# nelilepo/timetabling-ga-mpi-openmp

Hardware: AMD Instinct MI355X
Metric: fitness evals/sec (hcv+scv), pop 64K, 400-event instance; 1/2/4/8 GPUs (higher is better)
Workload: dtype i32; 1 GPU; med instance E=400 R=10 F=5 S=200 (seeded synthetic, medium01-size), population 65536 per GPU, one tt_eval (hcv+scv+feasible+penalty) per step; pop_per_gpu=65536, global_pop=65536, kernel=eval_tile5_w8, parallelism=dp1 (independent population shards)

## Files before the change

### timetabling-ga-mpi-openmp_amd/csrc/tt_eval.hip

```cpp
#include <algorithm>
#include <type_traits>
#include <utility>
#include <vector>

#include "tt_internal.h"

namespace ttga {

typedef __attribute__((address_space(4))) const uint32_t ConstU32;
typedef __attribute__((address_space(4))) const int32_t ConstI32;
typedef __attribute__((address_space(3))) unsigned long long LdsU64;


__device__ __forceinline__ int bcnt_acc(uint32_t x, int acc) {
    int r;
    asm("v_bcnt_u32_b32 %0, %1, %2" : "=v"(r) : "v"(x), "v"(acc));
    return r;
}
__device__ __forceinline__ int popc_acc(uint64_t x, int acc) {
    int r, t;
    asm("v_bcnt_u32_b32 %0, %1, %2" : "=v"(t) : "v"((uint32_t)x), "v"(acc));
    asm("v_bcnt_u32_b32 %0, %1, %2" : "=v"(r) : "v"((uint32_t)(x >> 32)), "v"(t));
    return r;
}
// ... 141 lines not shown
__device__ __forceinline__ int run_scv(const uint8_t* my, const uint32_t* p, int cnt) {
    constexpr int K = N <= 16 ? KMAX : 1;
    constexpr int ST = K * N / 2;
    const int steps = cnt / K;
    int sc = 0;
    if constexpr (KMAX == 1) {
        const ConstU32* q = (const ConstU32*)p;
        uint32_t cur[N / 2];
#pragma unroll
        for (int j = 0; j < N / 2; ++j) cur[j] = q[j];
        for (int i = 0; i < cnt; ++i) {
            const int in = i + 1 < cnt ? i + 1 : i;
            uint32_t nxt[N / 2];
#pragma unroll
            for (int j = 0; j < N / 2; ++j) nxt[j] = q[in * (N / 2) + j];
            uint32_t sl[N];
#pragma unroll
            for (int j = 0; j < N; ++j) sl[j] = my[(cur[j >> 1] >> (16 * (j & 1))) & 0xFFFFu];
            uint64_t m = 0;
#pragma unroll
            for (int j = 0; j < N; ++j) m |= 1ull << (sl[j] & 63);
            sc += mask_terms<GAP>(m);
#pragma unroll
            for (int j = 0; j < N / 2; ++j) cur[j] = nxt[j];
        }
        return sc;
    }
    const ConstU32* q = (const ConstU32*)p;
    if (steps > 0) {
        int i = 0;
        uint32_t ra[ST], rb[ST];
        sload_rec<ST>(q, ra);
        while (true) {
            sload_rec<ST>(q + (i + 1 < steps ? i + 1 : i) * ST, rb);
            sc += students_scv<N, K, GAP>(my, ra);
            keep_rec<ST>(rb);
            if (++i == steps) break;
            sload_rec<ST>(q + (i + 1 < steps ? i + 1 : i) * ST, ra);
            sc += students_scv<N, K, GAP>(my, rb);
            keep_rec<ST>(ra);
            if (++i == steps) break;
        }
    }
    if constexpr (K == 2) {
        if (cnt & 1) {
            uint32_t r[N / 2];
            sload_rec<N / 2>(q + steps * ST, r);
            sc += students_scv<N, 1, GAP>(my, r);
        }
    }
    return sc;
}
__device__ __noinline__ int run_scv_any(const uint8_t* my, const ConstU32* p, int cnt, int n, bool gap) {
    int sc = 0;
    for (int i = 0; i < cnt; ++i) {
        uint64_t m = 0;
        for (int j = 0; j < n / 2; ++j) {
            const uint32_t d = p[i * (n / 2) + j];
            m |= 1ull << (my[d & 0xFFFFu] & 63);
            m |= 1ull << (my[d >> 16] & 63);
        }
        sc += gap ? mask_scv_gap(m) : mask_scv(m);
    }
    return sc;
}
template <int KMAX, bool GAP = false>
__device__ __forceinline__ int lane_scv_runs(const uint8_t* my, const DevProblem& pb, int r0, int r1) {
    const ConstI32* runs = (const ConstI32*)pb.srun;
    int sc = 0;
    for (int k = r0; k < r1; ++k) {
        const int n = runs[4 * k], off = runs[4 * k + 1], cnt = runs[4 * k + 2];
        const uint32_t* p = pb.sid + off;
        switch (n) {
#define TT_RUN(N) case N: sc += run_scv<N, KMAX, GAP>(my, p, cnt); break;
            TT_RUN(2) TT_RUN(4) TT_RUN(6) TT_RUN(8) TT_RUN(10) TT_RUN(12) TT_RUN(14) TT_RUN(16)
            TT_RUN(18) TT_RUN(20) TT_RUN(22) TT_RUN(24) TT_RUN(26) TT_RUN(28) TT_RUN(30) TT_RUN(32)
#undef TT_RUN
            default: sc += run_scv_any(my, (const ConstU32*)p, cnt, n, GAP); break;
        }
    }
    return sc;
}

#ifndef TT_EVAL_ABLATE
#define TT_EVAL_ABLATE 0
#endif
__host__ __device__ inline int t5_cnt_bytes(int R) {
    return kSlots * ((R + 1) / 2) * 4;
}

struct Tile5Layout {
    int SP, WS;
    size_t tile_bytes, off_ws, off_part, bytes;
};

__host__ __device__ inline Tile5Layout tile5_layout(int E, int R, int NW, bool DB = false) {
    Tile5Layout L;
    int sp = (E + 1 + 3) & ~3;
    if (((sp >> 2) & 1) == 0) sp += 4;
    L.SP = sp;
    const int ew64 = (E + 63) / 64;
    const int cntb = t5_cnt_bytes(R);
    L.WS = (kSlots * ew64 * 8 + cntb + 15) & ~15;
    L.tile_bytes = ((size_t)64 * sp + 15) & ~(size_t)15;
    L.off_ws = (DB ? 2 : 1) * L.tile_bytes;
    L.off_part = L.off_ws + (size_t)NW * L.WS;
    L.bytes = L.off_part + 4 * (size_t)(NW * 64 + 64);
    return L;
}

template <int NW>
__device__ __forceinline__ void tile_dma(const uint8_t* src, uint8_t* dst, int np, int E, int SP, int wv, int lane) {
    const int qd = E >> 2;
    const __amdgpu_buffer_rsrc_t rs = __builtin_amdgcn_make_buffer_rsrc((void*)src, 0, np * E, 0x00020000);
    for (int r = wv; r < np; r += NW) {
        if (lane < qd)
            __builtin_amdgcn_raw_ptr_buffer_load_lds(rs, (__attribute__((address_space(3))) void*)(dst + r * SP), 4,
                                                     4 * lane, r * E, 0, 0);
        if (lane + 64 < qd)
            __builtin_amdgcn_raw_ptr_buffer_load_lds(rs, (__attribute__((address_space(3))) void*)(dst + r * SP + 256),
                                                     4, 4 * lane + 256, r * E, 0, 0);
    }
}

template <int NW>
__device__ __forceinline__ void image_dma(const uint8_t* img, int bytes, uint8_t* dst, int wv, int lane) {
    const __amdgpu_buffer_rsrc_t rs = __builtin_amdgcn_make_buffer_rsrc((void*)img, 0, bytes, 0x00020000);
    for (int k = wv; k < (bytes >> 8); k += NW)
        __builtin_amdgcn_raw_ptr_buffer_load_lds(rs, (__attribute__((address_space(3))) void*)(dst + 256 * k), 4,
                                                 4 * lane, 256 * k, 0, 0);
}

template <int EWC, int PK, int TP, typename PossT>
__device__ __forceinline__ void t5_load_inv(const uint8_t* img, int lane, uint64_t (*cup)[EWC], uint64_t* pcup,
                                            uint32_t* ps, PossT* poss, int* sn) {
    constexpr int F = TP == 1 ? EWC : EWC - 1;
    const uint64_t* c = (const uint64_t*)img + lane;
    const uint8_t* ev = img + 512 * t5_img_corr_rows(EWC, TP);
#pragma unroll
    for (int k = 0; k < t5_packed_rows(EWC, TP); ++k) pcup[k] = c[64 * (F * (F + 1) / 2 + k)];
#pragma unroll
    for (int r = 0; r < EWC; ++r) {
#pragma unroll
        for (int w = 0; w < EWC; ++w) cup[r][w] = (w >= r && w < F) ? c[64 * (r * F - r * (r - 1) / 2 + w - r)] : 0ull;
        if constexpr (PK == 1) {
            ps[r] = ((const uint32_t*)ev)[64 * r + lane];
        } else {
            poss[r] = ((const PossT*)ev)[64 * r + lane];
            sn[r] = ((const int*)(ev + EWC * 64 * sizeof(PossT)))[64 * r + lane];
        }
    }
}

#ifdef TT_T5_STAMP
constexpr int kT5Launches = 8, kT5MaxBlocks = 16384, kT5Words = 10;
__device__ unsigned long long g_t5_stamp[kT5Launches * kT5MaxBlocks * kT5Words];
#endif

__device__ __forceinline__ uint32_t mad_u16_hi(uint32_t a, uint32_t b, uint32_t c) {
    uint32_t d;
    asm("v_mad_u32_u16 %0, %1, %2, %3 op_sel:[0,1,0,0]" : "=v"(d) : "v"(a), "v"(b), "v"(c));
    return d;
}

constexpr uint32_t kT5ClrBias = 0x8000u;
constexpr size_t kT5ClrReach = 0x10000u + kT5ClrBias;
constexpr int t5_clear_max(int EWC, int PK) {
    return (kSlots * EWC * 8 + kSlots * (PK == 1 ? 8 : PK == 2 ? 16 : 32) * 4 + 15) / 256;
}
template <int MAXF>
__device__ __forceinline__ void t5_clear_pieces(uint32_t m0v, uint32_t skip) {
    uint32_t keep;
    asm volatile("s_mov_b32 %[keep], m0\n"
                 "s_mov_b32 m0, %[base]\n"
                 "s_getpc_b64 vcc\n"
                 "s_add_u32 vcc_lo, vcc_lo, %[skip]\n"
                 "s_addc_u32 vcc_hi, vcc_hi, 0\n"
                 "s_setpc_b64 vcc\n"
                 ".set tt_clr_k, %c[n]\n"
                 ".rept %c[n]\n"
                 ".set tt_clr_k, tt_clr_k-1\n"
                 "ds_write_addtid_b32 %[z] offset:tt_clr_k*256\n"
                 ".endr\n"
                 "s_branch .Ltt_clr_end%=\n"
                 ".set tt_clr_k, %c[n]\n"
                 ".rept %c[n]\n"
                 ".set tt_clr_k, tt_clr_k-1\n"
                 "ds_write_addtid_b32 %[z] offset:tt_clr_k*256+%c[bias]\n"
                 ".endr\n"
                 ".Ltt_clr_end%=:\n"
                 "s_mov_b32 m0, %[keep]\n"
                 "s_nop 0"
                 : [keep] "=&s"(keep)
                 : [base] "s"(m0v), [skip] "s"(skip), [z] "v"(0u), [n] "i"(MAXF), [bias] "i"(kT5ClrBias)
                 : "memory", "scc", "vcc");
}

constexpr int kT5PrioLane = 3;
constexpr uint32_t kT5PrioW = 0x00112233u;
template <int EWC, int NW, int PK, bool DB = false, int TP = 1>
__global__ __launch_bounds__(64 * NW, 4) void eval_tile5_kernel(DevProblem pb, const uint8_t* __restrict__ slot,
                                                              const uint8_t* __restrict__ room, int P,
                                                              int32_t* __restrict__ hcv_out,
                                                              int32_t* __restrict__ scv_out,
                                                              uint8_t* __restrict__ feas_out,
                                                              int32_t* __restrict__ pen_out, int ablate_arg) {
    extern __shared__ __attribute__((aligned(16))) uint8_t lds[];
    const int ablate = TT_EVAL_ABLATE ? ablate_arg : (ablate_arg & 3);
    constexpr int NT = 64 * NW;
#ifdef TT_T5_STAMP
    unsigned long long* st_rec =
        g_t5_stamp + ((size_t)((ablate_arg >> 8) & (kT5Launches - 1)) * kT5MaxBlocks + (blockIdx.x % kT5MaxBlocks)) * kT5Words;
    if (threadIdx.x == 0) {
        const unsigned long long t0 = __builtin_amdgcn_s_memrealtime();
        unsigned hw, xcc;
        asm volatile("s_getreg_b32 %0, hwreg(HW_REG_HW_ID)" : "=s"(hw));
        asm volatile("s_getreg_b32 %0, hwreg(HW_REG_XCC_ID)" : "=s"(xcc));
        st_rec[0] = t0;
        st_rec[1] = ((unsigned long long)xcc << 32) | hw;
    }
#endif
    const int E = pb.E, R = pb.R;
    const int lane = threadIdx.x & 63, wv = wave_id();
    const Tile5Layout L = tile5_layout(E, R, NW, DB);
    const int SP = L.SP;
    uint8_t* tile = lds;
    uint8_t* ws = lds + L.off_ws + (size_t)wv * L.WS;
    uint64_t* B = (uint64_t*)ws;
    uint32_t* cnt = (uint32_t*)(B + kSlots * EWC);
    int32_t* part = (int32_t*)(lds + L.off_part);
    int32_t* hq = part + NW * 64;
    const int tiles = (P + 63) / 64;
    const bool last_partial = E < 64 * EWC;
    const int RW = (R + 1) / 2;
    constexpr int CLRF = t5_clear_max(EWC, PK);
    const uint32_t ws_a = (uint32_t)__builtin_amdgcn_readfirstlane((int)lds_addr(ws));
    const bool ws_hi = ws_a >= 0x10000u;
    const uint32_t clr_m0 = ws_hi ? ws_a - kT5ClrBias : ws_a;
    const uint32_t clr_skip = 12u + 8u * (uint32_t)(CLRF - min(L.WS >> 8, CLRF)) + (ws_hi ? 8u * CLRF + 4u : 0u);

    using PossT = typename std::conditional<PK == 0, uint64_t, uint32_t>::type;
    uint64_t inv_cup[EWC][EWC];
    uint64_t inv_pcup[TP == 1 ? 1 : t5_packed_rows(EWC, TP)];
    PossT inv_poss[EWC];
    uint32_t inv_ps[EWC];
    int inv_sn[EWC];
    auto load_inv = [&](const uint8_t* img) { t5_load_inv<EWC, PK, TP, PossT>(img, lane, inv_cup, inv_pcup, inv_ps, inv_poss, inv_sn); };
    const bool img_lds = DB && (size_t)pb.t5_img_bytes <= L.tile_bytes;
    const ConstI32* ptab = (const ConstI32*)pb.srun_part;
    const int pbase = srun_part_base(NW);
    const int r0 = ptab[pbase + wv], r1 = ptab[pbase + wv + 1];
    const bool wide = (E & 15) == 0 && (((uintptr_t)slot) & 15) == 0;
    const int qpr = E >> 4;
    const uint32_t qinv = ((1u << 20) + (uint32_t)qpr - 1) / (uint32_t)max(qpr, 1);
    constexpr int TPL = 64 / TP;
    const uint32_t tcol = 64 * (EWC - 1) + ((lane & (TPL - 1)) + 64 * (EWC - 1) < E ? (lane & (TPL - 1)) : 0);
    const uint32_t pb0 = lds_addr(B) + 8 * (lane / TPL);

    if constexpr (DB) {
        if (threadIdx.x < 64) lds[threadIdx.x * SP + E] = 63;
        if (blockIdx.x < tiles)
            tile_dma<NW>(slot + (long)blockIdx.x * 64 * E, lds, (int)min(64L, (long)P - (long)blockIdx.x * 64), E, SP,
                         wv, lane);
        if (img_lds) {
            image_dma<NW>(pb.t5_img, pb.t5_img_bytes, lds + L.tile_bytes, wv, lane);
            asm volatile("s_waitcnt vmcnt(0)" ::: "memory");
            __syncthreads();
            load_inv(lds + L.tile_bytes);
            __syncthreads();
        } else {
            load_inv(pb.t5_img);
        }
        if (threadIdx.x < 64) lds[L.tile_bytes + threadIdx.x * SP + E] = 63;
    }
    auto stage = [&](const uint8_t* src, int np) {
        if (wide) {
            const uint4* s16 = (const uint4*)src;
#pragma unroll 2
            for (int w = threadIdx.x; w < np * qpr; w += NT) {
                const int r = (int)(((uint32_t)w * qinv) >> 20), c = w - r * qpr;
                const uint4 v = s16[w];
                uint32_t* d = (uint32_t*)(tile + r * SP + 16 * c);
                d[0] = v.x; d[1] = v.y; d[2] = v.z; d[3] = v.w;
            }
        } else {
#pragma unroll 1
            for (int r = wv; r < np; r += NW)
#pragma unroll 1
                for (int c = lane; c < E; c += 64) tile[r * SP + c] = src[(long)r * E + c];
        }
        if (threadIdx.x < 64) tile[threadIdx.x * SP + E] = 63;
    };
    if constexpr (!DB) {
        if (blockIdx.x < tiles)
            stage(slot + (long)blockIdx.x * 64 * E, (int)min(64L, (long)P - (long)blockIdx.x * 64));
        load_inv(pb.t5_img);
    }
    int it = 0;
    for (int tl = blockIdx.x; tl < tiles; tl += gridDim.x, ++it) {
        const long p0 = (long)tl * 64;
        const int np = (int)min((long)64, (long)P - p0);
        const uint8_t* src = slot + p0 * E;
        if constexpr (DB) {
            tile = lds + (it & 1) * L.tile_bytes;
            if (!(img_lds && it == 0)) {
                asm volatile("s_waitcnt vmcnt(0)" ::: "memory");
                __syncthreads();
            }
            const int tn = tl + gridDim.x;
            if (tn < tiles)
                tile_dma<NW>(slot + (long)tn * 64 * E, lds + ((it + 1) & 1) * L.tile_bytes,
                             (int)min(64L, (long)P - (long)tn * 64), E, SP, wv, lane);
        } else {
            if (it > 0) {
                __syncthreads();
                stage(src, np);
            }
            __syncthreads();
        }

        uint32_t lsp;
        asm volatile("v_mul_u32_u24 %0, %1, %2" : "=v"(lsp) : "v"(lane), "s"(SP));
        __builtin_amdgcn_s_setprio(kT5PrioLane);
        const int sc = (!(ablate & 1) && r0 < r1) ? lane_scv_runs<1>(tile + lsp, pb, r0, r1) : 0;
        part[wv * 64 + lane] = sc;

        const int nq = (ablate & 2) ? 0 : np;
        uint32_t pfn[EWC];
        const __amdgpu_buffer_rsrc_t rrs =
            __builtin_amdgcn_make_buffer_rsrc((void*)(room + p0 * E), 0, 64 * E, 0x00020000);
        auto load_row = [&](int q, uint32_t* dst) {
#pragma unroll
            for (int r = 0; r < EWC; ++r)
                dst[r] = (!last_partial || r < EWC - 1 || lane + 64 * r < E)
                             ? (uint32_t)__builtin_amdgcn_raw_buffer_load_b8(rrs, lane + 64 * r, q * E, 0)
                             : 0u;
        };
        if (wv < nq) load_row(wv, pfn);
        for (int q = wv; q < nq; q += NW) {
            const uint32_t pr = (kT5PrioW >> (4 * min((q - wv) / NW, 7))) & 3u;
            if (pr == 0) __builtin_amdgcn_s_setprio(0);
            else if (pr == 1) __builtin_amdgcn_s_setprio(1);
            else if (pr == 2) __builtin_amdgcn_s_setprio(2);
            else __builtin_amdgcn_s_setprio(3);
            uint32_t rv[EWC], sv[EWC];
#pragma unroll
            for (int r = 0; r < EWC; ++r) rv[r] = pfn[r];
            const uint8_t* rs = tile + q * SP;
#pragma unroll
            for (int r = 0; r < EWC; ++r)
                sv[r] = (!last_partial || r < EWC - 1 || lane + 64 * r < E) ? rs[lane + 64 * r] : 0u;
            uint32_t ts = 0;
            if constexpr (TP > 1) ts = rs[tcol];
            if (q + NW < nq) load_row(q + NW, pfn);
            uint32_t smax = 0, rmax = 0;
#pragma unroll
            for (int r = 0; r < EWC; ++r) { smax = max(smax, sv[r]); rmax = max(rmax, rv[r]); }
            const bool any_bad = wave_any(smax >= (uint32_t)kSlots || rmax >= (uint32_t)R);
            int h = 0, last = 0;
            if (!any_bad) {
                uint32_t row[EWC];
#pragma unroll
                for (int r = 0; r < EWC; ++r) row[r] = lds_addr(B) + __umul24(sv[r], (uint32_t)(EWC * 8));
                if (!(ablate & 32)) {
                    t5_clear_pieces<CLRF>(clr_m0, clr_skip);
                    *(uint32_t*)(ws + L.WS - 256 + 4 * lane) = 0u;
                }
                __builtin_amdgcn_fence(__ATOMIC_RELEASE, "wavefront");
                __builtin_amdgcn_wave_barrier();
                __builtin_amdgcn_fence(__ATOMIC_ACQUIRE, "wavefront");
#pragma unroll
                for (int r = 0; r < EWC; ++r) {
                    if (r < EWC - 1 || !last_partial || lane + 64 * r < E) {
                        const uint32_t s = sv[r], ro = rv[r];
                        if (!(ablate & 8))
                            __hip_atomic_fetch_or((LdsU64*)(uintptr_t)row[r] + r, 1ull << lane, __ATOMIC_RELAXED,
                                                  __HIP_MEMORY_SCOPE_AGENT);
                        if (!(ablate & 16)) {
                            uint32_t* c = (uint32_t*)((uint8_t*)cnt + ((__umul24(s, (uint32_t)(2 * RW)) + (ro & ~1u)) << 1));
                            const uint32_t sh = ro << 4;
                            h += (int)__builtin_amdgcn_ubfe(atomicAdd(c, 1u << (sh & 31u)), sh, 16);
                        }
                        const bool last_slot = (kLastSlotMask >> s) & 1ull;
                        if constexpr (PK == 1) {
                            h += (int)__builtin_amdgcn_ubfe(inv_ps[r], ro, 1);
                            last = (int)mad_u16_hi((uint32_t)(kLastSlotMask >> s) & 1u, inv_ps[r], (uint32_t)last);
                        } else {
                            h += (int)(((inv_poss[r] >> ro) & 1u) ^ 1u);
                            last += last_slot ? inv_sn[r] : 0;
                        }
                    }
                }
                __builtin_amdgcn_fence(__ATOMIC_RELEASE, "wavefront");
                __builtin_amdgcn_wave_barrier();
                __builtin_amdgcn_fence(__ATOMIC_ACQUIRE, "wavefront");
                if (!(ablate & 4)) {
                    if constexpr (TP == 1)
                        corr_words<0, EWC>(row, inv_cup, h);
                    else
                        corr_words_tp<0, EWC, TP>(row, pb0 + __umul24(ts, (uint32_t)(EWC * 8)), inv_cup, inv_pcup, h);
                }
                if (!wave_any(h >= 1024 || last >= 1024)) {
                    const uint32_t t = (uint32_t)wave_sum((h << 16) | last);
                    h = (int)(t >> 16);
                    last = (int)(t & 0xFFFFu);
                } else {
                    h = wave_sum(h);
                    last = wave_sum(last);
                }
                __builtin_amdgcn_fence(__ATOMIC_RELEASE, "wavefront");
                __builtin_amdgcn_wave_barrier();
                __builtin_amdgcn_fence(__ATOMIC_ACQUIRE, "wavefront");
            }
            if (lane == 0) {
                hq[q] = any_bad ? -1 : h;
                part[wv * 64 + q] += last;
            }
        }
        __syncthreads();
        if (wv == 0 && lane < np) {
            const long p = p0 + lane;
            const int h = hq[lane];
            if (h < 0) {
                hcv_out[p] = -1; scv_out[p] = -1; feas_out[p] = 0; pen_out[p] = -1;
            } else {
                int s2 = 0;
#pragma unroll
                for (int w = 0; w < NW; ++w) s2 += part[w * 64 + lane];
                hcv_out[p] = h;
                scv_out[p] = s2;
                feas_out[p] = h == 0 ? 1 : 0;
                pen_out[p] = h == 0 ? s2 : 1000000 + h;
            }
        }
    }
#ifdef TT_T5_STAMP
    if ((threadIdx.x & 63) == 0 && (threadIdx.x >> 6) < kT5Words - 2)
        st_rec[2 + (threadIdx.x >> 6)] = __builtin_amdgcn_s_memrealtime();
#endif
}

template <int NWL>
__global__ __launch_bounds__(64 * NWL) void eval_lanes_kernel(DevProblem pb, const uint8_t* __restrict__ slot, int P,
                                                              int32_t* __restrict__ scv_part) {
    extern __shared__ __attribute__((aligned(16))) uint8_t lds[];
    constexpr int NT = 64 * NWL;
    const int E = pb.E;
    const int lane = threadIdx.x & 63, wv = wave_id();
    int sp = (E + 1 + 3) & ~3;
    if (((sp >> 2) & 1) == 0) sp += 4;
    const int SP = sp;
    uint8_t* tile = lds;
    int32_t* part = (int32_t*)(lds + (((size_t)64 * SP + 15) & ~(size_t)15));
    const int tiles = (P + 63) / 64;
    const ConstI32* ptab = (const ConstI32*)pb.srun_part;
    const int pbase = srun_part_base(NWL);
    const int r0 = ptab[pbase + wv], r1 = ptab[pbase + wv + 1];
    const bool wide = (E & 15) == 0 && (((uintptr_t)slot) & 15) == 0;
    const int qpr = E >> 4;
    const uint64_t qinv = ((1ull << 32) + (uint64_t)qpr - 1) / (uint64_t)max(qpr, 1);

    for (int tl = blockIdx.x; tl < tiles; tl += gridDim.x) {
        const long p0 = (long)tl * 64;
        const int np = (int)min((long)64, (long)P - p0);
        __syncthreads();
        const uint8_t* src = slot + p0 * E;
        if (wide) {
            const uint4* s16 = (const uint4*)src;
#pragma unroll 2
            for (int w = threadIdx.x; w < np * qpr; w += NT) {
                const int r = (int)(((uint64_t)(uint32_t)w * qinv) >> 32), c = w - r * qpr;
                const uint4 v = s16[w];
                uint32_t* d = (uint32_t*)(tile + r * SP + 16 * c);
                d[0] = gap_slots4(v.x); d[1] = gap_slots4(v.y); d[2] = gap_slots4(v.z); d[3] = gap_slots4(v.w);
            }
        } else {
#pragma unroll 1
            for (int r = wv; r < np; r += NWL)
#pragma unroll 1
                for (int c = lane; c < E; c += 64) {
                    const uint8_t v = src[(long)r * E + c];
                    tile[r * SP + c] = gap_slot(v);
                }
        }
        if (threadIdx.x < 64) tile[threadIdx.x * SP + E] = 63;
        __syncthreads();
        const int sc = r0 < r1 ? lane_scv_runs<2, true>(tile + lane * SP, pb, r0, r1) : 0;
        part[wv * 64 + lane] = sc;
        __syncthreads();
        if (wv == 0 && lane < np) {
            int s2 = 0;
#pragma unroll
            for (int w = 0; w < NWL; ++w) s2 += part[w * 64 + lane];
            scv_part[p0 + lane] = s2;
        }
    }
}

struct CorrLayout {
    int NWV, BST, NB, EPL;
    size_t off_cnt, off_sl, WSI, off_acc, off_red, bytes;
};

__host__ __device__ inline CorrLayout corr_layout(int E, int R, int EW64, int NB) {
    CorrLayout L;
    const int pairs = (EW64 + 1) / 2;
    L.NWV = pairs < 16 ? pairs : 16;
    L.EPL = (E + 64 * L.NWV - 1) / (64 * L.NWV);
    L.BST = EW64 | 1;
    L.off_cnt = (size_t)kSlots * L.BST * 8;
    L.off_sl = L.off_cnt + (size_t)((kSlots * R + 1) / 2) * 4;
    L.WSI = (L.off_sl + (size_t)E + 15) & ~(size_t)15;
    L.NB = NB;
    L.off_acc = (size_t)NB * L.WSI;
    L.off_red = L.off_acc + (size_t)NB * 16;
    L.bytes = L.off_red + (size_t)NB * 2 * 64 * 4;
    return L;
}

constexpr int kCorrMaxEPL = 4;

template <int N, int OFF>
// ... 321 lines not shown
        std::vector<unsigned long long> z(sizeof(g_t5_stamp) / 8, 0ull);
        TT_HIP(hipMemcpyToSymbol(HIP_SYMBOL(g_t5_stamp), z.data(), sizeof(g_t5_stamp)));
    }
    return kT5Launches * kT5MaxBlocks;
}
#endif

extern "C" int tt_eval_variant(const tt_problem* p, const uint8_t* slot, const uint8_t* room, int P, int32_t* hcv,
                               int32_t* scv, uint8_t* feasible, int32_t* penalty, int variant, void* stream) {
    int rc = check_pop_args(p, P, slot, room);
    if (rc) return rc;
    if (P > 0 && (!hcv || !scv || !feasible || !penalty)) { set_error("null output buffer"); return TT_ERR_INVALID; }
    const int ablate = variant >> 4;
    variant &= 15;
    if (variant != 0 && variant != 2 && variant != 7 && variant != 8 && variant != 13) {
        set_error("unknown eval variant (0 auto, 2 block, 7/8 tile5, 13 wide)");
        return TT_ERR_INVALID;
    }
    if (P == 0) return TT_OK;
    rc = use_device(p);
    if (rc) return rc;
    hipStream_t st = (hipStream_t)stream;
    const int E = p->E, R = p->R;
    if (variant == 0) variant = auto_variant(p);
    if (variant == 13) {
        if (!wide_fits(p)) { set_error("instance outside the wide eval path"); return TT_ERR_LIMIT; }
        const int EW64 = p->dev.EW64;
        const int tiles = (P + 63) / 64;
        {
            const size_t lds_l = lanes_lds_bytes(E);
            auto launch_l = [&](auto kern) -> int {
                int per_cu = 0;
                TT_HIP(hipOccupancyMaxActiveBlocksPerMultiprocessor(&per_cu, kern, 1024, lds_l));
                per_cu = std::min(per_cu, lds_resident_limit(lds_l));
                const int grid = std::min(tiles, std::max(1, per_cu) * p->num_cus);
                hipLaunchKernelGGL(kern, dim3(grid), dim3(1024), lds_l, st, p->dev, slot, P, scv);
                return TT_OK;
            };
            rc = launch_l(eval_lanes_kernel<16>);
            if (rc) return rc;
        }
        if (ablate & 4) return check_hip(hipGetLastError(), "tt_eval launch");
        const int NB = corr_nb(E, R, EW64);
        const CorrLayout CL = corr_layout(E, R, EW64, NB);
        auto launch = [&](auto kern) -> int {
            int per_cu = 0;
            TT_HIP(hipOccupancyMaxActiveBlocksPerMultiprocessor(&per_cu, kern, 64 * CL.NWV, CL.bytes));
            per_cu = std::min(per_cu, lds_resident_limit(CL.bytes));
            const long batches = ((long)P + NB - 1) / NB;
            const int grid = (int)std::min<long>(batches, (long)std::max(1, per_cu) * p->num_cus);
            hipLaunchKernelGGL(kern, dim3(grid), dim3(64 * CL.NWV), CL.bytes, st, p->dev, slot, room, P, hcv, scv,
                               feasible, penalty, ablate);
            return TT_OK;
        };
        if (CL.EPL <= 2)
            rc = NB == 8 ? launch(eval_corr_kernel<8, 2>) : NB == 4 ? launch(eval_corr_kernel<4, 2>) : launch(eval_corr_kernel<2, 2>);
        else
            rc = NB == 8 ? launch(eval_corr_kernel<8, kCorrMaxEPL>)
                 : NB == 4 ? launch(eval_corr_kernel<4, kCorrMaxEPL>) : launch(eval_corr_kernel<2, kCorrMaxEPL>);
        if (rc) return rc;
    } else if (variant == 7 || variant == 8) {
        const int NW = variant == 7 ? 4 : 8;
        const Tile5Layout L0 = tile5_layout(E, R, NW, false), L1 = tile5_layout(E, R, NW, true);
        const bool db_ok = (E & 3) == 0 && (((uintptr_t)slot) & 3) == 0 && L1.bytes <= 160 * 1024 &&
                           L1.off_part <= kT5ClrReach;
        if (p->dev.EW64 > 7 || L0.bytes > 160 * 1024 || L0.off_part > kT5ClrReach || E > 32767) {
            set_error("instance too large for the tile5 kernel");
            return TT_ERR_LIMIT;
        }
        const int pk = t5_pk(R, p->max_sn), tp = t5_tp(E);
        const int tiles = (P + 63) / 64;
        auto occupancy = [&](auto kern, size_t bytes, bool two) -> int {
            std::atomic<int>& c = const_cast<tt_problem*>(p)->t5_occ[NW == 8][two];
            int per_cu = c.load(std::memory_order_relaxed);
            if (per_cu >= 0) return per_cu;
            if (hipOccupancyMaxActiveBlocksPerMultiprocessor(&per_cu, kern, 64 * NW, bytes) != hipSuccess) {
                (void)hipGetLastError();
                return 0;
            }
            per_cu = std::min(per_cu, lds_resident_limit(bytes));
            c.store(per_cu, std::memory_order_relaxed);
            return per_cu;
        };
        auto launch = [&](auto kern, size_t bytes, bool two) -> int {
            const int per_cu = occupancy(kern, bytes, two);
            const bool persist = (ablate & 64) || (two && !(ablate & 128));
            const int grid = persist ? std::min(tiles, std::max(1, per_cu) * p->num_cus) : tiles;
            hipLaunchKernelGGL(kern, dim3(grid), dim3(64 * NW), bytes, st, p->dev, slot, room, P, hcv, scv,
                               feasible, penalty, ablate);
            return TT_OK;
        };
#define TT_T5U(EWC, NWV, PKV, TPV)                                                                                 \
    {                                                                                                              \
        const bool db = db_ok && occupancy(eval_tile5_kernel<EWC, NWV, PKV, true, TPV>, L1.bytes, true) >=         \
                                     occupancy(eval_tile5_kernel<EWC, NWV, PKV, false, TPV>, L0.bytes, false);     \
        rc = db ? launch(eval_tile5_kernel<EWC, NWV, PKV, true, TPV>, L1.bytes, true)                              \
                : launch(eval_tile5_kernel<EWC, NWV, PKV, false, TPV>, L0.bytes, false);                           \
    }
#define TT_T5P(EWC, NWV, PKV) \
    if (EWC > 1 && tp == 4) { TT_T5U(EWC, NWV, PKV, (EWC > 1 ? 4 : 1)) } else { TT_T5U(EWC, NWV, PKV, 1) }
#define TT_T5N(EWC, NWV) \
    if (pk == 1) { TT_T5P(EWC, NWV, 1) } else if (pk == 2) { TT_T5P(EWC, NWV, 2) } else { TT_T5P(EWC, NWV, 0) }
#define TT_T5(EWC)                                                      \
    case EWC:                                                           \
        if (NW == 4) { TT_T5N(EWC, 4) } else { TT_T5N(EWC, 8) }         \
        break;
        switch (p->dev.EW64) {
            TT_T5(1) TT_T5(2) TT_T5(3) TT_T5(4) TT_T5(5) TT_T5(6) TT_T5(7)
            default: rc = TT_ERR_LIMIT; break;
        }
#undef TT_T5
#undef TT_T5N
#undef TT_T5P
#undef TT_T5U
        if (rc) return rc;
    } else {
        const size_t lds = block_lds_bytes(E, R);
        if (lds > 160 * 1024) { set_error("instance too large for the block kernel"); return TT_ERR_LIMIT; }
        hipLaunchKernelGGL(eval_block_kernel, dim3(P), dim3(kBlockThreads), lds, st, p->dev, slot, room, P, hcv,
                           scv, feasible, penalty);
    }
    return check_hip(hipGetLastError(), "tt_eval launch");
}

extern "C" int tt_eval(const tt_problem* p, const uint8_t* slot, const uint8_t* room, int P, int32_t* hcv,
                       int32_t* scv, uint8_t* feasible, int32_t* penalty, void* stream) {
    return tt_eval_variant(p, slot, room, P, hcv, scv, feasible, penalty, 0, stream);
}
```

Measured before the change: 1.036 billion evals/s.

## Add paired-tile tile5 kernel that evaluates soft constraints for two tiles per pass

Adds a PAIR variant of the double-buffered 8-wave tile5 kernel. It keeps two population tiles in LDS at a fixed distance, so each student-run pass reads both tiles and builds two slot masks at once, reusing the decoded student lists and index loads. The per-wave hard-constraint body moves into an include file that both variants share. The pair path also reschedules DMA and write-out around the two tiles and uses LDS atomics for the accumulators. This adds layout complexity, extra LDS and workgroup atomics, and more register pressure from the doubled gather buffers.

```diff
diff --git a/timetabling-ga-mpi-openmp_amd/csrc/tt_eval.hip b/timetabling-ga-mpi-openmp_amd/csrc/tt_eval.hip
--- a/timetabling-ga-mpi-openmp_amd/csrc/tt_eval.hip
+++ b/timetabling-ga-mpi-openmp_amd/csrc/tt_eval.hip
@@ -247,6 +247,93 @@
     return sc;
 }
 
+constexpr int kT5PairChunk = 3;
+template <int N, int D, bool GAP>
+__device__ __forceinline__ void student_scv2(const uint8_t* my, const uint32_t* r, int& sca, int& scb) {
+    constexpr int CH = kT5PairChunk, NCH = (N + CH - 1) / CH;
+    uint64_t ma = 0, mb = 0;
+    uint32_t sa[2][CH], sb[2][CH];
+    auto gather = [&](int c) __attribute__((always_inline)) {
+#pragma unroll
+        for (int j = c * CH; j < c * CH + CH && j < N; ++j) {
+            const uint8_t* q = my + ((r[j >> 1] >> (16 * (j & 1))) & 0xFFFFu);
+            sa[c & 1][j - c * CH] = q[0];
+            sb[c & 1][j - c * CH] = q[D];
+        }
+    };
+    gather(0);
+#pragma unroll
+    for (int c = 0; c < NCH; ++c) {
+        if (c + 1 < NCH) gather(c + 1);
+        asm volatile("" ::: "memory");
+        __builtin_amdgcn_sched_barrier(0);
+#pragma unroll
+        for (int j = c * CH; j < c * CH + CH && j < N; ++j) {
+            ma |= 1ull << (sa[c & 1][j - c * CH] & 63);
+            mb |= 1ull << (sb[c & 1][j - c * CH] & 63);
+        }
+        asm volatile("" : "+v"(ma), "+v"(mb) : : "memory");
+        __builtin_amdgcn_sched_barrier(0);
+    }
+    sca += mask_terms<GAP>(ma);
+    scb += mask_terms<GAP>(mb);
+}
+template <int N, int D, bool GAP>
+__device__ __forceinline__ void run_scv2(const uint8_t* my, const uint32_t* p, int cnt, int& sca, int& scb) {
+    const ConstU32* q = (const ConstU32*)p;
+    uint32_t cur[N / 2];
+#pragma unroll
+    for (int j = 0; j < N / 2; ++j) cur[j] = q[j];
+    for (int i = 0; i < cnt; ++i) {
+        const int in = i + 1 < cnt ? i + 1 : i;
+        uint32_t nxt[N / 2];
+#pragma unroll
+        for (int j = 0; j < N / 2; ++j) nxt[j] = q[in * (N / 2) + j];
+        student_scv2<N, D, GAP>(my, cur, sca, scb);
+        keep_rec<N / 2>(nxt);
+#pragma unroll
+        for (int j = 0; j < N / 2; ++j) cur[j] = nxt[j];
+    }
+}
+template <int D>
+__device__ __noinline__ int2 run_scv_any2(const uint8_t* my, const ConstU32* p, int cnt, int n, bool gap) {
+    int2 sc = make_int2(0, 0);
+    for (int i = 0; i < cnt; ++i) {
+        uint64_t ma = 0, mb = 0;
+        for (int j = 0; j < n / 2; ++j) {
+            const uint32_t d = p[i * (n / 2) + j];
+            const uint8_t *q0 = my + (d & 0xFFFFu), *q1 = my + (d >> 16);
+            ma |= 1ull << (q0[0] & 63);
+            mb |= 1ull << (q0[D] & 63);
+            ma |= 1ull << (q1[0] & 63);
+            mb |= 1ull << (q1[D] & 63);
+        }
+        sc.x += gap ? mask_scv_gap(ma) : mask_scv(ma);
+        sc.y += gap ? mask_scv_gap(mb) : mask_scv(mb);
+    }
+    return sc;
+}
+template <int D, bool GAP = false>
+__device__ __forceinline__ void lane_scv_runs2(const uint8_t* my, const DevProblem& pb, int r0, int r1, int& sca,
+                                               int& scb) {
+    const ConstI32* runs = (const ConstI32*)pb.srun;
+    for (int k = r0; k < r1; ++k) {
+        const int n = runs[4 * k], off = runs[4 * k + 1], cnt = runs[4 * k + 2];
+        const uint32_t* p = pb.sid + off;
+        switch (n) {
+#define TT_RUN(N) case N: run_scv2<N, D, GAP>(my, p, cnt, sca, scb); break;
+            TT_RUN(2) TT_RUN(4) TT_RUN(6) TT_RUN(8) TT_RUN(10) TT_RUN(12) TT_RUN(14) TT_RUN(16)
+            TT_RUN(18) TT_RUN(20) TT_RUN(22) TT_RUN(24) TT_RUN(26) TT_RUN(28) TT_RUN(30) TT_RUN(32)
+#undef TT_RUN
+            default: {
+                const int2 s = run_scv_any2<D>(my, (const ConstU32*)p, cnt, n, GAP);
+                sca += s.x;
+                scb += s.y;
+            } break;
+        }
+    }
+}
+
 #ifndef TT_EVAL_ABLATE
 #define TT_EVAL_ABLATE 0
 #endif
@@ -272,6 +359,28 @@
     L.off_part = L.off_ws + (size_t)NW * L.WS;
     L.bytes = L.off_part + 4 * (size_t)(NW * 64 + 64);
     return L;
+}
+
+__host__ __device__ constexpr int t5_pair_dist(int EWC) { return 4096 * EWC + 2048; }
+constexpr int kT5PairAcc = 4 * 4 * 64;
+struct Tile5PairLayout {
+    int kgap;
+    size_t off_ws_hi, off_acc, bytes;
+};
+__host__ __device__ inline Tile5PairLayout tile5_pair_layout(const Tile5Layout& L, int EWC, int NW) {
+    Tile5PairLayout Q;
+    const size_t gap = (size_t)t5_pair_dist(EWC) - L.tile_bytes;
+    Q.kgap = (int)(gap / (size_t)L.WS < (size_t)NW ? gap / (size_t)L.WS : (size_t)NW);
+    const size_t used = (size_t)Q.kgap * L.WS;
+    Q.off_ws_hi = (size_t)t5_pair_dist(EWC) + L.tile_bytes;
+    Q.bytes = Q.off_ws_hi + (size_t)(NW - Q.kgap) * L.WS;
+    if (gap - used >= (size_t)kT5PairAcc) {
+        Q.off_acc = L.tile_bytes + used;
+    } else {
+        Q.off_acc = Q.bytes;
+        Q.bytes += kT5PairAcc;
+    }
+    return Q;
 }
 
 template <int NW>
@@ -363,7 +472,9 @@
 
 constexpr int kT5PrioLane = 3;
 constexpr uint32_t kT5PrioW = 0x00112233u;
-template <int EWC, int NW, int PK, bool DB = false, int TP = 1>
+constexpr uint32_t kT5PairPrioA = 0x33333333u, kT5PairPrioB = 0x00001111u;
+constexpr int kT5PairPrioLane = 2;
+template <int EWC, int NW, int PK, bool DB = false, int TP = 1, bool PAIR = false>
 __global__ __launch_bounds__(64 * NW, 4) void eval_tile5_kernel(DevProblem pb, const uint8_t* __restrict__ slot,
                                                               const uint8_t* __restrict__ room, int P,
                                                               int32_t* __restrict__ hcv_out,
@@ -389,12 +500,21 @@
     const int lane = threadIdx.x & 63, wv = wave_id();
     const Tile5Layout L = tile5_layout(E, R, NW, DB);
     const int SP = L.SP;
+    static_assert(!PAIR || (DB && NW == 8), "the paired form: two tile buffers, 8 waves");
     uint8_t* tile = lds;
     uint8_t* ws = lds + L.off_ws + (size_t)wv * L.WS;
+    int32_t* part = (int32_t*)(lds + L.off_part);
+    int32_t* hq = part + NW * 64;
+    size_t buf1 = L.tile_bytes;
+    if constexpr (PAIR) {
+        const Tile5PairLayout Q = tile5_pair_layout(L, EWC, NW);
+        ws = lds + (wv < Q.kgap ? L.tile_bytes + (size_t)wv * L.WS : Q.off_ws_hi + (size_t)(wv - Q.kgap) * L.WS);
+        part = (int32_t*)(lds + Q.off_acc);
+        hq = part + 2 * 64;
+        buf1 = t5_pair_dist(EWC);
+    }
     uint64_t* B = (uint64_t*)ws;
     uint32_t* cnt = (uint32_t*)(B + kSlots * EWC);
-    int32_t* part = (int32_t*)(lds + L.off_part);
-    int32_t* hq = part + NW * 64;
     const int tiles = (P + 63) / 64;
     const bool last_partial = E < 64 * EWC;
     const int RW = (R + 1) / 2;
@@ -424,19 +544,22 @@
 
     if constexpr (DB) {
         if (threadIdx.x < 64) lds[threadIdx.x * SP + E] = 63;
+        if constexpr (PAIR) {
+            if (threadIdx.x < 2 * 64) part[threadIdx.x] = 0;
+        }
         if (blockIdx.x < tiles)
             tile_dma<NW>(slot + (long)blockIdx.x * 64 * E, lds, (int)min(64L, (long)P - (long)blockIdx.x * 64), E, SP,
                          wv, lane);
         if (img_lds) {
-            image_dma<NW>(pb.t5_img, pb.t5_img_bytes, lds + L.tile_bytes, wv, lane);
+            image_dma<NW>(pb.t5_img, pb.t5_img_bytes, lds + buf1, wv, lane);
             asm volatile("s_waitcnt vmcnt(0)" ::: "memory");
             __syncthreads();
-            load_inv(lds + L.tile_bytes);
+            load_inv(lds + buf1);
             __syncthreads();
         } else {
             load_inv(pb.t5_img);
         }
-        if (threadIdx.x < 64) lds[L.tile_bytes + threadIdx.x * SP + E] = 63;
+        if (threadIdx.x < 64) lds[buf1 + threadIdx.x * SP + E] = 63;
     }
     auto stage = [&](const uint8_t* src, int np) {
         if (wide) {
@@ -461,6 +584,8 @@
             stage(slot + (long)blockIdx.x * 64 * E, (int)min(64L, (long)P - (long)blockIdx.x * 64));
         load_inv(pb.t5_img);
     }
+
+    if constexpr (!PAIR) {
     int it = 0;
     for (int tl = blockIdx.x; tl < tiles; tl += gridDim.x, ++it) {
         const long p0 = (long)tl * 64;
@@ -490,98 +615,13 @@
         const int sc = (!(ablate & 1) && r0 < r1) ? lane_scv_runs<1>(tile + lsp, pb, r0, r1) : 0;
         part[wv * 64 + lane] = sc;
 
-        const int nq = (ablate & 2) ? 0 : np;
-        uint32_t pfn[EWC];
-        const __amdgpu_buffer_rsrc_t rrs =
-            __builtin_amdgcn_make_buffer_rsrc((void*)(room + p0 * E), 0, 64 * E, 0x00020000);
-        auto load_row = [&](int q, uint32_t* dst) {
-#pragma unroll
-            for (int r = 0; r < EWC; ++r)
-                dst[r] = (!last_partial || r < EWC - 1 || lane + 64 * r < E)
-                             ? (uint32_t)__builtin_amdgcn_raw_buffer_load_b8(rrs, lane + 64 * r, q * E, 0)
-                             : 0u;
-        };
-        if (wv < nq) load_row(wv, pfn);
-        for (int q = wv; q < nq; q += NW) {
-            const uint32_t pr = (kT5PrioW >> (4 * min((q - wv) / NW, 7))) & 3u;
-            if (pr == 0) __builtin_amdgcn_s_setprio(0);
-            else if (pr == 1) __builtin_amdgcn_s_setprio(1);
-            else if (pr == 2) __builtin_amdgcn_s_setprio(2);
-            else __builtin_amdgcn_s_setprio(3);
-            uint32_t rv[EWC], sv[EWC];
-#pragma unroll
-            for (int r = 0; r < EWC; ++r) rv[r] = pfn[r];
-            const uint8_t* rs = tile + q * SP;
-#pragma unroll
-            for (int r = 0; r < EWC; ++r)
-                sv[r] = (!last_partial || r < EWC - 1 || lane + 64 * r < E) ? rs[lane + 64 * r] : 0u;
-            uint32_t ts = 0;
-            if constexpr (TP > 1) ts = rs[tcol];
-            if (q + NW < nq) load_row(q + NW, pfn);
-            uint32_t smax = 0, rmax = 0;
-#pragma unroll
-            for (int r = 0; r < EWC; ++r) { smax = max(smax, sv[r]); rmax = max(rmax, rv[r]); }
-            const bool any_bad = wave_any(smax >= (uint32_t)kSlots || rmax >= (uint32_t)R);
-            int h = 0, last = 0;
-            if (!any_bad) {
-                uint32_t row[EWC];
-#pragma unroll
-                for (int r = 0; r < EWC; ++r) row[r] = lds_addr(B) + __umul24(sv[r], (uint32_t)(EWC * 8));
-                if (!(ablate & 32)) {
-                    t5_clear_pieces<CLRF>(clr_m0, clr_skip);
-                    *(uint32_t*)(ws + L.WS - 256 + 4 * lane) = 0u;
-                }
-                __builtin_amdgcn_fence(__ATOMIC_RELEASE, "wavefront");
-                __builtin_amdgcn_wave_barrier();
-                __builtin_amdgcn_fence(__ATOMIC_ACQUIRE, "wavefront");
-#pragma unroll
-                for (int r = 0; r < EWC; ++r) {
-                    if (r < EWC - 1 || !last_partial || lane + 64 * r < E) {
-                        const uint32_t s = sv[r], ro = rv[r];
-                        if (!(ablate & 8))
-                            __hip_atomic_fetch_or((LdsU64*)(uintptr_t)row[r] + r, 1ull << lane, __ATOMIC_RELAXED,
-                                                  __HIP_MEMORY_SCOPE_AGENT);
-                        if (!(ablate & 16)) {
-                            uint32_t* c = (uint32_t*)((uint8_t*)cnt + ((__umul24(s, (uint32_t)(2 * RW)) + (ro & ~1u)) << 1));
-                            const uint32_t sh = ro << 4;
-                            h += (int)__builtin_amdgcn_ubfe(atomicAdd(c, 1u << (sh & 31u)), sh, 16);
-                        }
-                        const bool last_slot = (kLastSlotMask >> s) & 1ull;
-                        if constexpr (PK == 1) {
-                            h += (int)__builtin_amdgcn_ubfe(inv_ps[r], ro, 1);
-                            last = (int)mad_u16_hi((uint32_t)(kLastSlotMask >> s) & 1u, inv_ps[r], (uint32_t)last);
-                        } else {
-                            h += (int)(((inv_poss[r] >> ro) & 1u) ^ 1u);
-                            last += last_slot ? inv_sn[r] : 0;
-                        }
-                    }
-                }
-                __builtin_amdgcn_fence(__ATOMIC_RELEASE, "wavefront");
-                __builtin_amdgcn_wave_barrier();
-                __builtin_amdgcn_fence(__ATOMIC_ACQUIRE, "wavefront");
-                if (!(ablate & 4)) {
-                    if constexpr (TP == 1)
-                        corr_words<0, EWC>(row, inv_cup, h);
-                    else
-                        corr_words_tp<0, EWC, TP>(row, pb0 + __umul24(ts, (uint32_t)(EWC * 8)), inv_cup, inv_pcup, h);
-                }
-                if (!wave_any(h >= 1024 || last >= 1024)) {
-                    const uint32_t t = (uint32_t)wave_sum((h << 16) | last);
-                    h = (int)(t >> 16);
-                    last = (int)(t & 0xFFFFu);
-                } else {
-                    h = wave_sum(h);
-                    last = wave_sum(last);
-                }
-                __builtin_amdgcn_fence(__ATOMIC_RELEASE, "wavefront");
-                __builtin_amdgcn_wave_barrier();
-                __builtin_amdgcn_fence(__ATOMIC_ACQUIRE, "wavefront");
-            }
-            if (lane == 0) {
-                hq[q] = any_bad ? -1 : h;
-                part[wv * 64 + q] += last;
-            }
-        }
+#define T5W_SCHED kT5PrioW
+#define T5W_HQ hq
+#define T5W_LAST(q, v) part[wv * 64 + (q)] += (v)
+#include "tt_eval_t5_wave.inc"
+#undef T5W_SCHED
+#undef T5W_HQ
+#undef T5W_LAST
         __syncthreads();
         if (wv == 0 && lane < np) {
             const long p = p0 + lane;
@@ -599,10 +639,88 @@
             }
         }
     }
+    } else {
+        constexpr int D = t5_pair_dist(EWC);
+        auto write_out = [&](long p0, int np, int t) {
+            if (wv == 0 && lane < np) {
+                const long p = p0 + lane;
+                const int h = hq[64 * t + lane], s2 = part[64 * t + lane];
+                part[64 * t + lane] = 0;
+                hcv_out[p] = h < 0 ? -1 : h;
+                scv_out[p] = h < 0 ? -1 : s2;
+                feas_out[p] = h == 0 ? 1 : 0;
+                pen_out[p] = h < 0 ? -1 : h == 0 ? s2 : 1000000 + h;
+            }
+        };
+        if (!img_lds) {
+            asm volatile("s_waitcnt vmcnt(0)" ::: "memory");
+            __syncthreads();
+        }
+        for (int ta = blockIdx.x; ta < tiles; ta += 2 * gridDim.x) {
+            const int tb = ta + gridDim.x;
+            const bool has_b = tb < tiles;
+            const long p0a = (long)ta * 64, p0b = (long)tb * 64;
+            const int npa = (int)min((long)64, (long)P - p0a), npb = has_b ? (int)min((long)64, (long)P - p0b) : 0;
+            if (has_b) tile_dma<NW>(slot + p0b * E, lds + D, npb, E, SP, wv, lane);
+#define T5W_LAST(q, v) __hip_atomic_fetch_add(T5W_ACC + (q), (v), __ATOMIC_RELAXED, __HIP_MEMORY_SCOPE_WORKGROUP)
+#define T5W_ACC part
+            {
+                const uint8_t* tile = lds;
+                const long p0 = p0a;
+                const int np = npa;
+#define T5W_SCHED kT5PairPrioA
+#define T5W_HQ hq
+#include "tt_eval_t5_wave.inc"
+#undef T5W_SCHED
+#undef T5W_HQ
+#undef T5W_ACC
+            }
+            asm volatile("s_waitcnt vmcnt(0)" ::: "memory");
+            __syncthreads();
+
+            uint32_t lsp;
+            asm volatile("v_mul_u32_u24 %0, %1, %2" : "=v"(lsp) : "v"(lane), "s"(SP));
+            __builtin_amdgcn_s_setprio(kT5PairPrioLane);
+            int sca = 0, scb = 0;
+            if (!(ablate & 1) && r0 < r1) lane_scv_runs2<D>(lds + lsp, pb, r0, r1, sca, scb);
+            __hip_atomic_fetch_add(part + lane, sca, __ATOMIC_RELAXED, __HIP_MEMORY_SCOPE_WORKGROUP);
+            if (has_b) __hip_atomic_fetch_add(part + 64 + lane, scb, __ATOMIC_RELAXED, __HIP_MEMORY_SCOPE_WORKGROUP);
+            __syncthreads();
+
+            const int tn = ta + 2 * gridDim.x;
+            if (tn < tiles)
+                tile_dma<NW>(slot + (long)tn * 64 * E, lds, (int)min(64L, (long)P - (long)tn * 64), E, SP, wv, lane);
+            write_out(p0a, npa, 0);
+            if (has_b) {
+                const uint8_t* tile = lds + D;
+                const long p0 = p0b;
+                const int np = npb;
+                int32_t* const hqb = hq + 64;
+#define T5W_SCHED kT5PairPrioB
+#define T5W_HQ hqb
+#define T5W_ACC (part + 64)
+#include "tt_eval_t5_wave.inc"
+#undef T5W_SCHED
+#undef T5W_HQ
+#undef T5W_ACC
+            }
+#undef T5W_LAST
+            asm volatile("s_waitcnt vmcnt(0)" ::: "memory");
+            __syncthreads();
+            if (has_b) write_out(p0b, npb, 1);
+        }
+    }
 #ifdef TT_T5_STAMP
     if ((threadIdx.x & 63) == 0 && (threadIdx.x >> 6) < kT5Words - 2)
         st_rec[2 + (threadIdx.x >> 6)] = __builtin_amdgcn_s_memrealtime();
 #endif
+}
+
+typedef void (*T5Kern)(DevProblem, const uint8_t*, const uint8_t*, int, int32_t*, int32_t*, uint8_t*, int32_t*, int);
+template <int EWC, int NW, int PK, int TP>
+inline T5Kern t5_pair_kernel() {
+    if constexpr (NW == 8) return eval_tile5_kernel<EWC, NW, PK, true, TP, true>;
+    else return nullptr;
 }
 
 template <int NWL>
@@ -1090,10 +1208,23 @@
             c.store(per_cu, std::memory_order_relaxed);
             return per_cu;
         };
-        auto launch = [&](auto kern, size_t bytes, bool two) -> int {
+        const Tile5PairLayout Q1 = tile5_pair_layout(L1, p->dev.EW64, NW);
+        auto launch = [&](auto kern, size_t bytes, bool two, T5Kern kern2 = nullptr) -> int {
             const int per_cu = occupancy(kern, bytes, two);
+            if (kern2 && two && !(ablate & (128 | 4096)) && Q1.bytes <= 160 * 1024 &&
+                Q1.off_ws_hi + (size_t)(NW - Q1.kgap) * L1.WS <= kT5ClrReach &&
+                lds_resident_limit(Q1.bytes) >= per_cu) {
+                int grid = std::min(tiles, std::max(1, per_cu) * p->num_cus);
+                if (ablate & 2048) grid = std::min(grid, 2);
+                if (tiles >= 2 * grid) {
+                    hipLaunchKernelGGL(kern2, dim3(grid), dim3(64 * NW), Q1.bytes, st, p->dev, slot, room, P, hcv,
+                                       scv, feasible, penalty, ablate);
+                    return TT_OK;
+                }
+            }
             const bool persist = (ablate & 64) || (two && !(ablate & 128));
-            const int grid = persist ? std::min(tiles, std::max(1, per_cu) * p->num_cus) : tiles;
+            int grid = persist ? std::min(tiles, std::max(1, per_cu) * p->num_cus) : tiles;
+            if (persist && (ablate & 2048)) grid = std::min(grid, 2);
             hipLaunchKernelGGL(kern, dim3(grid), dim3(64 * NW), bytes, st, p->dev, slot, room, P, hcv, scv,
                                feasible, penalty, ablate);
             return TT_OK;
@@ -1102,7 +1233,8 @@
     {                                                                                                              \
         const bool db = db_ok && occupancy(eval_tile5_kernel<EWC, NWV, PKV, true, TPV>, L1.bytes, true) >=         \
                                      occupancy(eval_tile5_kernel<EWC, NWV, PKV, false, TPV>, L0.bytes, false);     \
-        rc = db ? launch(eval_tile5_kernel<EWC, NWV, PKV, true, TPV>, L1.bytes, true)                              \
+        rc = db ? launch(eval_tile5_kernel<EWC, NWV, PKV, true, TPV>, L1.bytes, true,                              \
+                         t5_pair_kernel<EWC, NWV, PKV, TPV>())                                                     \
                 : launch(eval_tile5_kernel<EWC, NWV, PKV, false, TPV>, L0.bytes, false);                           \
     }
 #define TT_T5P(EWC, NWV, PKV) \
diff --git a/timetabling-ga-mpi-openmp_amd/csrc/tt_eval_t5_wave.inc b/timetabling-ga-mpi-openmp_amd/csrc/tt_eval_t5_wave.inc
--- /dev/null
+++ b/timetabling-ga-mpi-openmp_amd/csrc/tt_eval_t5_wave.inc
@@ -0,0 +1,92 @@
+        const int nq = (ablate & 2) ? 0 : np;
+        uint32_t pfn[EWC];
+        const __amdgpu_buffer_rsrc_t rrs =
+            __builtin_amdgcn_make_buffer_rsrc((void*)(room + p0 * E), 0, 64 * E, 0x00020000);
+        auto load_row = [&](int q, uint32_t* dst) {
+#pragma unroll
+            for (int r = 0; r < EWC; ++r)
+                dst[r] = (!last_partial || r < EWC - 1 || lane + 64 * r < E)
+                             ? (uint32_t)__builtin_amdgcn_raw_buffer_load_b8(rrs, lane + 64 * r, q * E, 0)
+                             : 0u;
+        };
+        if (wv < nq) load_row(wv, pfn);
+        for (int q = wv; q < nq; q += NW) {
+            const uint32_t pr = (T5W_SCHED >> (4 * min((q - wv) / NW, 7))) & 3u;
+            if (pr == 0) __builtin_amdgcn_s_setprio(0);
+            else if (pr == 1) __builtin_amdgcn_s_setprio(1);
+            else if (pr == 2) __builtin_amdgcn_s_setprio(2);
+            else __builtin_amdgcn_s_setprio(3);
+            uint32_t rv[EWC], sv[EWC];
+#pragma unroll
+            for (int r = 0; r < EWC; ++r) rv[r] = pfn[r];
+            const uint8_t* rs = tile + q * SP;
+#pragma unroll
+            for (int r = 0; r < EWC; ++r)
+                sv[r] = (!last_partial || r < EWC - 1 || lane + 64 * r < E) ? rs[lane + 64 * r] : 0u;
+            uint32_t ts = 0;
+            if constexpr (TP > 1) ts = rs[tcol];
+            if (q + NW < nq) load_row(q + NW, pfn);
+            uint32_t smax = 0, rmax = 0;
+#pragma unroll
+            for (int r = 0; r < EWC; ++r) { smax = max(smax, sv[r]); rmax = max(rmax, rv[r]); }
+            const bool any_bad = wave_any(smax >= (uint32_t)kSlots || rmax >= (uint32_t)R);
+            int h = 0, last = 0;
+            if (!any_bad) {
+                uint32_t row[EWC];
+#pragma unroll
+                for (int r = 0; r < EWC; ++r) row[r] = lds_addr(B) + __umul24(sv[r], (uint32_t)(EWC * 8));
+                if (!(ablate & 32)) {
+                    t5_clear_pieces<CLRF>(clr_m0, clr_skip);
+                    *(uint32_t*)(ws + L.WS - 256 + 4 * lane) = 0u;
+                }
+                __builtin_amdgcn_fence(__ATOMIC_RELEASE, "wavefront");
+                __builtin_amdgcn_wave_barrier();
+                __builtin_amdgcn_fence(__ATOMIC_ACQUIRE, "wavefront");
+#pragma unroll
+                for (int r = 0; r < EWC; ++r) {
+                    if (r < EWC - 1 || !last_partial || lane + 64 * r < E) {
+                        const uint32_t s = sv[r], ro = rv[r];
+                        if (!(ablate & 8))
+                            __hip_atomic_fetch_or((LdsU64*)(uintptr_t)row[r] + r, 1ull << lane, __ATOMIC_RELAXED,
+                                                  __HIP_MEMORY_SCOPE_AGENT);
+                        if (!(ablate & 16)) {
+                            uint32_t* c = (uint32_t*)((uint8_t*)cnt + ((__umul24(s, (uint32_t)(2 * RW)) + (ro & ~1u)) << 1));
+                            const uint32_t sh = ro << 4;
+                            h += (int)__builtin_amdgcn_ubfe(atomicAdd(c, 1u << (sh & 31u)), sh, 16);
+                        }
+                        const bool last_slot = (kLastSlotMask >> s) & 1ull;
+                        if constexpr (PK == 1) {
+                            h += (int)__builtin_amdgcn_ubfe(inv_ps[r], ro, 1);
+                            last = (int)mad_u16_hi((uint32_t)(kLastSlotMask >> s) & 1u, inv_ps[r], (uint32_t)last);
+                        } else {
+                            h += (int)(((inv_poss[r] >> ro) & 1u) ^ 1u);
+                            last += last_slot ? inv_sn[r] : 0;
+                        }
+                    }
+                }
+                __builtin_amdgcn_fence(__ATOMIC_RELEASE, "wavefront");
+                __builtin_amdgcn_wave_barrier();
+                __builtin_amdgcn_fence(__ATOMIC_ACQUIRE, "wavefront");
+                if (!(ablate & 4)) {
+                    if constexpr (TP == 1)
+                        corr_words<0, EWC>(row, inv_cup, h);
+                    else
+                        corr_words_tp<0, EWC, TP>(row, pb0 + __umul24(ts, (uint32_t)(EWC * 8)), inv_cup, inv_pcup, h);
+                }
+                if (!wave_any(h >= 1024 || last >= 1024)) {
+                    const uint32_t t = (uint32_t)wave_sum((h << 16) | last);
+                    h = (int)(t >> 16);
+                    last = (int)(t & 0xFFFFu);
+                } else {
+                    h = wave_sum(h);
+                    last = wave_sum(last);
+                }
+                __builtin_amdgcn_fence(__ATOMIC_RELEASE, "wavefront");
+                __builtin_amdgcn_wave_barrier();
+                __builtin_amdgcn_fence(__ATOMIC_ACQUIRE, "wavefront");
+            }
+            if (lane == 0) {
+                T5W_HQ[q] = any_bad ? -1 : h;
+                T5W_LAST(q, last);
+            }
+        }
```

After: 1.023 billion evals/s. -1.2%, worse.
